# parsaeskandar/pangenome-index

Hardware: AMD Instinct MI355X
Metric: find_mems reads/sec (150 bp batch) (higher is better)
Workload: dtype u64

## Files before the change

pangenome-index_amd/csrc/pgx_image.h:

```cpp
#ifndef PGX_IMAGE_H
#define PGX_IMAGE_H

#include <stdint.h>

#define PGX_IMAGE_LAYOUT 1u

#define PGX_BLOCK_BYTES 64
#define PGX_BLOCK_RUNS 16
#define PGX_RUN_LEN_BITS 12
#define PGX_RUN_LEN_MAX 4095u
#define PGX_COUNT_BITS 40
#define PGX_DIR_MAX_SHIFT 12
#define PGX_IMAGE_RL 0u
#define PGX_IMAGE_DENSE 1u
#define PGX_IMAGE_DENSE2 2u
#define PGX_D2_SYMS 384u
#define PGX_D2_BLOCK_BYTES 128u
#define PGX_PAIRS_SYMS 96u
#define PGX_PAIRS_BLOCK_BYTES 128u
#define PGX_PAIRS_STRIDE64 64u
#define PGX_SB_MAX 64u
#define PGX_D2_SB_SHIFT 22u
#define PGX_PAIRS_SB_SHIFT 24u

#define PGX_EXT_CV(e) ((e) & 7u)
#define PGX_EXT_V(e) (((e) >> 3) & 7u)
#define PGX_EXT_M(e) (((e) >> 6) & 0x3FFFFu)
#define PGX_EXT_KILL(e) (((e) >> 24) & 1u)
#define PGX_EXT_MAKE(cv, v, m, kill) \
    ((uint32_t)(cv) | ((uint32_t)(v) << 3) | ((uint32_t)(m) << 6) | ((uint32_t)(kill) << 24))

typedef struct {
    uint64_t n;
    uint64_t C[8];
    uint32_t ext_tab[512];
    uint32_t slot_code[8];
    uint32_t sigma;
    uint32_t excl_mask;
    uint32_t dir_shift;
    uint32_t n_blocks;
    uint64_t dir_entries;
    uint64_t n_tag_runs;
    uint64_t tag_dir_entries;
    uint32_t tag_dir_shift;
    uint32_t has_tags;
    uint32_t mode;
    uint32_t count_supported;
    uint32_t cnt_tab[256];
    uint32_t image_kind;
    uint32_t has_pairs;
    uint32_t pair_t2[32];
    uint32_t pair_runs;
    uint32_t reserved1;
    uint32_t wide;
    uint32_t d2_sb_shift, pairs_sb_shift;
    uint32_t n_sb2, n_sbp;
    uint32_t pairs_stride;
    uint64_t pair_t2w[32];
} PgxConsts;

#define PGX_NO_POSITION (~(uint64_t)0)
typedef struct {
    uint64_t n;
    uint64_t n_runs;
    uint64_t n_last;
    uint64_t max_length;
    uint64_t rdir_entries, ldir_entries;
    uint32_t rdir_shift, ldir_shift;
} PgxLocConsts;

// ... 2 lines not shown
```

pangenome-index_amd/csrc/pgx_index.cpp:

```cpp
#include <algorithm>
#include <cstdio>
#include <cstdlib>
#include <array>
#include <cstring>
#include <memory>
#include <mutex>
#include <thread>

#include "pgx_host.hpp"

namespace pgx {

static thread_local std::string g_last_error;
void set_last_error(const std::string &m) { g_last_error = m; }
const std::string &last_error() { return g_last_error; }

static inline unsigned bytecode_len(uint64_t v) {
    unsigned k = 1;
    while (v > 0x7F) { v >>= 7; k++; }
    return k;
}

void RiFile::parse(const uint8_t *p, uint64_t n) {
    ByteReader r(p, n);
// ... 306 lines not shown
static void build_dense_image(const RiFile &ri, HostImage &img) {
    PgxConsts &c = img.consts;
    const uint64_t nb = (c.n >> 6) + 1;
    if (nb >> 32) throw Error(PGX_ERR_UNSUPPORTED, "BWT too long for the dense image");
    img.blocks.assign(nb * PGX_BLOCK_BYTES, 0);
    img.bstart.clear();
    img.dir.assign(1, 0);
    img.blow.clear();
    uint32_t *dw = reinterpret_cast<uint32_t *>(img.blocks.data());
    uint64_t c6[6] = {0, 0, 0, 0, 0, 0};
    auto put_header = [&](uint64_t b) {
        uint32_t *h = dw + b * 16;
        for (int i = 0; i < 6; i++) h[i] = (uint32_t)c6[i];
        for (int i = 0; i < 4; i++) h[6] |= (uint32_t)((c6[i] >> 32) & 0xFF) << (8 * i);
        h[7] = (uint32_t)((c6[4] >> 32) & 0xFF) | ((uint32_t)((c6[5] >> 32) & 0xFF) << 8);
    };
    uint64_t pos = 0, n_runs = 0;
    put_header(0);
    for (const auto &blk : ri.blocks)
        for (const auto &ru : blk.runs) {
            n_runs++;
            const uint32_t code = ru.first;
            uint64_t left = ru.second;
            while (left) {
                const uint64_t b = pos >> 6;
                const uint32_t off = (uint32_t)(pos & 63);
                const uint64_t take = std::min<uint64_t>(left, 64 - off);
                const uint64_t bits = (take == 64 ? ~0ull : ((1ull << take) - 1ull)) << off;
                uint32_t *h = dw + b * 16;
                for (int p = 0; p < 3; p++)
                    if ((code >> p) & 1u) {
                        h[8 + 2 * p] |= (uint32_t)bits;
                        h[9 + 2 * p] |= (uint32_t)(bits >> 32);
                    }
                c6[code] += take;
                left -= take;
                pos += take;
                if ((pos & 63) == 0) put_header(pos >> 6);
            }
        }
    if (pos != c.n) throw Error(PGX_ERR_FORMAT, "FastLocate: run lengths do not add up to the BWT size");
    img.n_runs = n_runs;
    c.n_blocks = (uint32_t)nb;
    c.dir_shift = 0;
    c.dir_entries = 1;
    c.image_kind = PGX_IMAGE_DENSE;
}

static uint32_t sb_shift_for(uint64_t nb, uint32_t want) {
    uint32_t sh = want;
    while (((nb - 1) >> sh) + 1 > PGX_SB_MAX) sh++;
    return sh;
}
static void build_dense2_image(const RiFile &ri, HostImage &img, bool wide, uint32_t sb_shift_want) {
    PgxConsts &c = img.consts;
    if ((c.n >> 32) && !wide) throw Error(PGX_ERR_UNSUPPORTED, "BWT too long for the narrow dense2 image");
    const uint64_t nb = c.n / PGX_D2_SYMS + 1;
    if (nb >> 32) throw Error(PGX_ERR_UNSUPPORTED, "BWT too long for the dense2 image");
    const uint32_t sb_shift = wide ? sb_shift_for(nb, sb_shift_want) : 31u;
    if (wide && (PGX_D2_SYMS << sb_shift) > (1ull << 31)) throw Error(PGX_ERR_UNSUPPORTED, "BWT too long for the wide dense2 image (more than PGX_SB_MAX superblocks)");
    const uint64_t n_sb = wide ? ((nb - 1) >> sb_shift) + 1 : 1;
    img.sbase2.assign(n_sb * 8, 0);
    uint64_t base[6] = {0, 0, 0, 0, 0, 0};
    img.blocks.assign(nb * PGX_D2_BLOCK_BYTES, 0);
    img.bstart.clear();
    img.dir.assign(1, 0);
    img.blow.clear();
    img.exc.clear();
    uint32_t *dw = reinterpret_cast<uint32_t *>(img.blocks.data());
    uint64_t c6[6] = {0, 0, 0, 0, 0, 0};
    static const int hdr_slot[6] = {-1, 0, 1, 2, 4, 3};
    static const int two_bit[6] = {0, 0, 1, 2, 0, 3};
    auto put_header = [&](uint64_t b) {
        uint32_t *h = dw + b * 32;
        if (wide && (b & ((1ull << sb_shift) - 1)) == 0) {
            uint64_t *sb = img.sbase2.data() + (b >> sb_shift) * 8;
            uint64_t sum = 0;
            for (int i = 1; i < 6; i++) { base[i] = c6[i]; sb[hdr_slot[i]] = c6[i]; sum += c6[i]; }
            sb[5] = sum;
        }
        for (int i = 1; i < 6; i++) h[hdr_slot[i]] = (uint32_t)(c6[i] - base[i]);
        if (img.exc.size() >> 24) throw Error(PGX_ERR_UNSUPPORTED, "too many exception runs for the dense2 image");
        h[5] = (uint32_t)img.exc.size();
    };
    auto set_bits = [](uint32_t *words, uint32_t lo, uint32_t hi) {
        for (uint32_t w = lo >> 5; w <= ((hi - 1) >> 5); w++) {
            const uint32_t a = std::max(lo, w << 5) & 31u, e = std::min(hi, (w + 1) << 5) - (w << 5);
            words[w] |= (e == 32 ? 0xFFFFFFFFu : ((1u << e) - 1u)) & ~((1u << a) - 1u);
        }
    };
    auto finish_block = [&](uint64_t b) {
        uint32_t *h = dw + b * 32;
        uint64_t sub = 0;
        uint32_t n0 = 0, n1 = 0, n3 = 0;
        for (int s = 0; s < 2; s++) {
            for (int k = 0; k < 4; k++) {
                const uint32_t a = h[8 + 8 * s + k], d = h[12 + 8 * s + k];
                n0 += (uint32_t)__builtin_popcount(a); n1 += (uint32_t)__builtin_popcount(d); n3 += (uint32_t)__builtin_popcount(a & d);
            }
            sub |= ((uint64_t)n0 | ((uint64_t)n1 << 9) | ((uint64_t)n3 << 18)) << (27 * s);
        }
        h[6] = (uint32_t)sub; h[7] = (uint32_t)(sub >> 32);
    };
    uint64_t pos = 0, n_runs = 0;
    put_header(0);
    for (const auto &blk : ri.blocks)
        for (const auto &ru : blk.runs) {
            n_runs++;
            const uint32_t code = ru.first;
            uint64_t left = ru.second;
            while (left) {
                const uint64_t b = pos / PGX_D2_SYMS;
                const uint32_t off = (uint32_t)(pos % PGX_D2_SYMS);
                const uint64_t take = std::min<uint64_t>(left, PGX_D2_SYMS - off);
                uint32_t *h = dw + b * 32;
                const int tb = two_bit[code];
                if (tb)
                    for (uint32_t i = off; i < off + (uint32_t)take;) {
                        uint32_t *sb = h + 8 + 8 * (i >> 7);
                        const uint32_t lo = i & 127u, hi = std::min<uint32_t>(128u, lo + (off + (uint32_t)take - i));
                        if (tb & 1) set_bits(sb, lo, hi);
                        if (tb & 2) set_bits(sb + 4, lo, hi);
                        i += hi - lo;
                    }
                if (code == 0 || code == 4) {
                    const uint32_t kind = code == 4 ? 1u : 0u;
                    if ((h[5] >> 24) && (img.exc.back() >> 18) == kind && (img.exc.back() & 511u) + ((img.exc.back() >> 9) & 511u) == off)
                        img.exc.back() += (uint32_t)take << 9;
                    else {
                        img.exc.push_back(off | ((uint32_t)take << 9) | (kind << 18));
                        h[5] += 1u << 24;
                    }
                }
                c6[code] += take;
                left -= take;
                pos += take;
                if (pos % PGX_D2_SYMS == 0) { finish_block(b); put_header(pos / PGX_D2_SYMS); }
            }
        }
    if (pos != c.n) throw Error(PGX_ERR_FORMAT, "FastLocate: run lengths do not add up to the BWT size");
    finish_block(nb - 1);
    if (img.exc.empty()) img.exc.push_back(0);
    img.n_runs = n_runs;
    c.n_blocks = (uint32_t)nb;
    c.dir_shift = 0;
    c.dir_entries = 1;
    c.image_kind = PGX_IMAGE_DENSE2;
    c.wide = wide ? 1u : 0u;
    c.d2_sb_shift = sb_shift;
    c.n_sb2 = (uint32_t)n_sb;
}

static bool build_pairs_image(const RiFile &ri, HostImage &img, bool wide, uint32_t sb_shift_want, uint32_t stride) {
    if (stride != PGX_PAIRS_SYMS && stride != PGX_PAIRS_STRIDE64) return false;
    PgxConsts &c = img.consts;
// ... 196 lines not shown
        if (const char *e = std::getenv("PGX_IMAGE")) {
            const std::string v(e);
            force = v == "dense" ? PGX_MODE_IMAGE_DENSE : v == "dense2" ? PGX_MODE_IMAGE_DENSE2 : v == "rl" ? PGX_MODE_IMAGE_RL : v == "pairs" ? PGX_MODE_IMAGE_PAIRS : 0u;
            if (v == "wide" || v == "wide-pairs") { wide = true; force = PGX_MODE_IMAGE_PAIRS; }
            if (v == "wide-dense2") { wide = true; force = PGX_MODE_IMAGE_DENSE2; }
        }
    if (force & (force - 1)) throw Error(PGX_ERR_ARG, "pgx_index_open: more than one image layout forced");
    if (wide && (force & (PGX_MODE_IMAGE_RL | PGX_MODE_IMAGE_DENSE))) throw Error(PGX_ERR_ARG, "pgx_index_open: PGX_MODE_IMAGE_WIDE goes with dense2 / pairs only");
    if (wide && !force) force = PGX_MODE_IMAGE_PAIRS;
    const bool fits_wide = c.n < ((uint64_t)PGX_SB_MAX << 30);
    if (force & (PGX_MODE_IMAGE_DENSE | PGX_MODE_IMAGE_DENSE2 | PGX_MODE_IMAGE_PAIRS)) {
        if (!can) throw Error(PGX_ERR_UNSUPPORTED, "dense image: not available for a legacy-layout index without N in COMPAT mode");
        if ((force & (PGX_MODE_IMAGE_DENSE2 | PGX_MODE_IMAGE_PAIRS)) && (c.n >> 32)) {
            if (!fits_wide) throw Error(PGX_ERR_UNSUPPORTED, "dense2 image: BWT too long");
            wide = true;
        }
        if (force & PGX_MODE_IMAGE_PAIRS) pairs = wide && !(mode_bits & PGX_MODE_IMAGE_PAIRS) && !std::getenv("PGX_IMAGE") ? 1 : 2;
        return (force & PGX_MODE_IMAGE_DENSE) ? PGX_IMAGE_DENSE : PGX_IMAGE_DENSE2;
    }
    if ((force & PGX_MODE_IMAGE_RL) || !can) return PGX_IMAGE_RL;
    const uint64_t dense_blocks = (c.n >> 6) + 1;
    if (dense_blocks * 80 + 16 <= 48 * 1024) return PGX_IMAGE_DENSE;
    const uint64_t dense_bytes0 = dense_blocks * PGX_BLOCK_BYTES;
    if (dense_bytes0 <= (224ull << 20)) { pairs = (c.n >> 32) ? 0 : 1; return PGX_IMAGE_DENSE; }
    if (!(c.n >> 32)) { pairs = 1; return PGX_IMAGE_DENSE2; }
    if (fits_wide) { pairs = 1; wide = true; return PGX_IMAGE_DENSE2; }
    uint64_t runs = 0;
    for (const auto &b : ri.blocks) runs += b.runs.size();
    const uint64_t dense_bytes = dense_blocks * PGX_BLOCK_BYTES, rl_bytes = (runs / PGX_BLOCK_RUNS + 1) * (PGX_BLOCK_BYTES + 4);
    const uint64_t cache = 192ull << 20;
    return (rl_bytes > cache && dense_bytes <= (64ull << 30)) ? PGX_IMAGE_DENSE : PGX_IMAGE_RL;
}

void build_rank_image(const RiFile &ri, uint32_t mode_bits, HostImage &img) {
    const uint32_t mode = mode_bits & PGX_MODE_MASK;
    PgxConsts &c = img.consts;
    std::memset(&c, 0, sizeof c);
    c.n = ri.sequence_size;
    c.mode = mode;
    build_ext_tables(ri, mode, c);
    build_count_table(ri, mode, c);
    int pairs = 0;
    bool wide = false;
    const uint32_t kind = choose_image(ri, mode_bits, c, pairs, wide);
    img.pairs.clear(); img.sbase2.clear(); img.pbase.clear();
    uint32_t sh2 = PGX_D2_SB_SHIFT, shp = PGX_PAIRS_SB_SHIFT;
    if (const char *e = std::getenv("PGX_SB_SHIFT")) { sh2 = (uint32_t)std::min<unsigned long>(std::strtoul(e, nullptr, 10), PGX_D2_SB_SHIFT); shp = sh2 + 2; }
    uint32_t pstride = (2 * c.n <= (64ull << 30)) ? PGX_PAIRS_STRIDE64 : PGX_PAIRS_SYMS;
    if (const char *e = std::getenv("PGX_PAIRS_STRIDE")) {
        const unsigned long v = std::strtoul(e, nullptr, 10);
        if (v == PGX_PAIRS_SYMS) pstride = PGX_PAIRS_SYMS;
        else if (v == PGX_PAIRS_STRIDE64) pstride = PGX_PAIRS_STRIDE64;
    }
    if (kind == PGX_IMAGE_DENSE) {
        build_dense_image(ri, img);
        if (pairs) (void)build_pairs_image(ri, img, false, shp, pstride);
        return;
    }
    if (kind == PGX_IMAGE_DENSE2) {
        build_dense2_image(ri, img, wide, sh2);
        if (pairs && !build_pairs_image(ri, img, wide, shp, pstride) && pairs == 2)
            throw Error(PGX_ERR_UNSUPPORTED, "pairs image: the index does not qualify (extension tables of a COMPAT quirk, or too many N / endmarker runs)");
        return;
    }
    const bool refine = c.excl_mask != 0;
    img.blocks.clear();
    img.bstart.clear();
    uint64_t c6[6] = {0, 0, 0, 0, 0, 0};
    uint64_t head[6];
    std::vector<std::pair<uint8_t, uint32_t>> ent;
    uint64_t pos = 0, block_pos = 0, E = 0, n_runs = 0;
    auto open_block = [&]() {
        for (int i = 0; i < 6; i++) head[i] = (c.excl_mask >> i) & 1 ? E : c6[i];
        block_pos = pos;
        ent.clear();
    };
    auto close_block = [&]() {
        if (ent.empty()) return;
        put_block(img.blocks, head, ent);
        img.bstart.push_back(block_pos);
        ent.clear();
    };
    open_block();
    for (uint64_t b = 0; b < ri.blocks.size(); b++) {
        if (refine) {
            close_block();
            E = ri.blocks[b].cum[0];
            open_block();
        }
        for (auto &ru : ri.blocks[b].runs) {
            n_runs++;
            uint64_t left = ru.second;
            while (left) {
                if (!ent.empty() && ent.back().first == ru.first && ent.back().second < PGX_RUN_LEN_MAX) {
                    uint32_t add = (uint32_t)std::min<uint64_t>(left, PGX_RUN_LEN_MAX - ent.back().second);
                    ent.back().second += add;
                    left -= add; pos += add; c6[ru.first] += add;
                    continue;
                }
                if (ent.size() == PGX_BLOCK_RUNS) { close_block(); open_block(); }
                uint32_t take = (uint32_t)std::min<uint64_t>(left, PGX_RUN_LEN_MAX);
                ent.emplace_back(ru.first, take);
                left -= take; pos += take; c6[ru.first] += take;
            }
        }
    }
    close_block();
    if (img.bstart.empty()) {
        uint64_t z[6] = {0};
        put_block(img.blocks, z, {});
        img.bstart.push_back(0);
    }
    img.n_runs = n_runs;
// ... 394 lines not shown
```

pangenome-index_amd/csrc/pgx_pairs_kernels.hip:

```cpp
#include <hip/hip_runtime.h>
#include <stdint.h>

#include <type_traits>

#include "pgx_device.h"
#include "pgx_rank_device.h"
#include "pgx_slots_device.h"

#ifndef PGX_PAIRS_PACKED_WAVES
#define PGX_PAIRS_PACKED_WAVES 5
#endif
#ifndef PGX_LCE_WAVES
#define PGX_LCE_WAVES PGX_FM_WAVES_PER_SIMD
#endif
#ifndef PGX_LCE_ENTRY_CAP
#define PGX_LCE_ENTRY_CAP 3u
#endif
#define PGX_PK_GROUP 12u

__device__ __forceinline__ uint32_t pgx_window_byte(uint64_t w0, uint64_t w1, uint64_t a) {
    return (uint32_t)(((a & 8ull) ? w1 : w0) >> (8u * (uint32_t)(a & 7ull))) & 0xFFu;
}
__device__ __forceinline__ uint32_t pgx_packed_seed_index(const uint32_t *s_rd, uint32_t rd_stride, uint32_t q, int32_t K) {
    const uint32_t w0 = s_rd[(q >> 4) * rd_stride + threadIdx.x], w1 = s_rd[((q >> 4) + 1u) * rd_stride + threadIdx.x];
// ... 432 lines not shown
                const int32_t ta = (int32_t)relA - 32 * h, tb = (int32_t)relB - 32 * h;
                const uint32_t mP = ta >= 32 ? 0xFFFFFFFFu : (ta > 0 ? ((1u << ta) - 1u) : 0u);
                const uint32_t mR = (tb >= 32 ? 0xFFFFFFFFu : (tb > 0 ? ((1u << tb) - 1u) : 0u)) & ~mP;
                const uint32_t x = PX[h], y = PY[h], u = PU[h], v = PV[h];
                const uint32_t m1 = (x ^ i0) & (y ^ i1);
                const uint32_t g1 = (y & ua) | (x & (y | va) & wa);
                const uint32_t q2 = m1 & (u ^ j0) & (v ^ j1);
                const uint32_t g2 = m1 & ((v & ub) | (u & (v | vb) & wb));
                e1p += __popc(m1 & mP); e2p += __popc(q2 & mP);
                e1r += __popc(m1 & mR); g1r += __popc(g1 & mR); e2r += __popc(q2 & mR); g2r += __popc(g2 & mR);
            }
            pos_t a01 = (pos_t)(row.x + row.y + row.z + row.w + pts + e1p);
            pos_t a02 = (pos_t)((t2 == 0u ? row.x : (t2 == 1u ? row.y : (t2 == 2u ? row.z : row.w))) + e2p);
            if (WIDE) {
                const uint64_t *pb = s_pb + (size_t)((bfirst + pend) >> pa.pairs_sb_shift) * 24u;
                a01 += (pos_t)pb[16u + t1];
                a02 += (pos_t)pb[4u * t1 + t2];
            }
            const bool straddle = endrel > SYMS, far = endrel > STRIDE + SYMS;
            const uint32_t over = endrel - SYMS;
            const bool cont2 = !pend && straddle && over <= (hs.y >> 24), cont1 = !pend && straddle && !cont2 && over <= (hs.z >> 24);
            const bool cont = cont1 || cont2;
            if (cont) {
                const uint32_t l1 = (PX[2] >> 31) | ((PY[2] >> 31) << 1), l2 = (PU[2] >> 31) | ((PV[2] >> 31) << 1);
                e1r += l1 == t1 ? over : 0u;
                g1r += l1 > t1 ? over : 0u;
                e2r += (cont2 && l1 == t1 && l2 == t2) ? over : 0u;
                g2r += (cont2 && l1 == t1 && l2 > t2) ? over : 0u;
            }
            const bool bail = !fr && (flagged || (far && !cont));
            const bool wait = !fr && !pend && straddle && !bail && !cont;
#ifdef PGX_FM_STATS
            st_wait += wait ? 1ull : 0ull;
#endif
            if (wait) {
                X0 = e1r | (g1r << 8) | (e2r << 16) | (g2r << 24); X0e = a01; X0f = a02;
                pend = 1u;
            } else {
                const uint32_t Xp = pend ? X0 : 0u;
                const uint32_t c1 = (Xp & 0xFFu) + e1r, w1 = ((Xp >> 8) & 0xFFu) + g1r, c2 = ((Xp >> 16) & 0xFFu) + e2r, w2 = (Xp >> 24) + g2r;
                const pos_t r1 = pend ? X0e : a01, r2 = pend ? X0f : a02;
                pend = 0u;
                pos_t s1 = reg1 ? (pos_t)c1 : (pos_t)0;
                pos_t k1 = r1 + s_C[PGX_EXT_V(e1)], q1v = kq + (pos_t)w1;
                if (bail) {
                    const uint64_t q0 = (uint64_t)p0 > (uint64_t)n ? (uint64_t)n : (uint64_t)p0, q1 = (uint64_t)p1 > (uint64_t)n ? (uint64_t)n : (uint64_t)p1;
                    uint64_t A0 = 0, A1 = 0, B0 = 0, B1 = 0;
                    PgxDevImage img = {};
                    img.blocks = PGX_PAIRS_COLD(blocks); img.exc = PGX_PAIRS_COLD(exc); img.sbase2 = PGX_PAIRS_COLD(sbase2); img.d2_sb_shift = PGX_PAIRS_COLD(d2_sb_shift);
#pragma unroll 1
                    for (int it = 0; it < 2; it++) {
                        const uint64_t q = it ? q1 : q0;
                        uint64_t a, bq;
                        if (WIDE) pgx_dense2w_rank(img, q, PGX_EXT_CV(e1), PGX_EXT_M(e1), a, bq);
                        else if (pa.dense == 1) {
                            const PgxDenseBlk db = pgx_dense_load<false>(img, nullptr, q);
                            pgx_dense_rank(db, q, PGX_EXT_CV(e1), PGX_EXT_M(e1), a, bq);
                        } else pgx_dense2_rank(img, (uint32_t)q, PGX_EXT_CV(e1), PGX_EXT_M(e1), a, bq);
                        A1 = a; B1 = bq;
                        if (!it) { A0 = a; B0 = bq; }
                    }
                    const uint64_t dB = B1 - B0;
                    {
                        const unsigned long long here = __ballot(true);
                        if (lane == (int)__ffsll((long long)here) - 1) {
                            atomicAdd(PGX_PAIRS_COLD(ctr) + PGX_CTR_REDO, (unsigned long long)__popcll(here));
                            atomicAdd(PGX_PAIRS_COLD(ctr) + PGX_CTR_PAIRS_LINES, 2ull * (unsigned long long)__popcll(here));
                        }
                    }
                    const bool none = PGX_EXT_KILL(e1) || A0 >= A1;
                    s1 = none ? (pos_t)0 : (pos_t)(A1 - A0);
                    k1 = (pos_t)A0 + s_C[PGX_EXT_V(e1)];
                    q1v = kq + (pos_t)dB;
                }
                if (fr) { const uint4 f = s_fe[PACKED ? (at_end ? 4u : ((byte >> 1) & 3u)) : byte]; k1 = ent_k(f); q1v = ent_q(f); s1 = ent_s(f); }
                const bool small1 = s1 == 0u || s1 < mo || mo_huge;
                const uint32_t sdepth = se.w >> 24;
                const pos_t se_s = ent_s(se);
                const bool seed_alive = seed_lane && se_s != 0u && se_s >= mo && !mo_huge;
                const bool seed_dead = seed_lane && se_s == 0u && sdepth != PGX_SEED_UNUSABLE && mo <= 1u;
                const bool do2 = (fr ? (at_end && rem2 && have2 && !seed_alive && !seed_dead) : (two && !bail && !cont1)) && !small1;
                pos_t s2 = (pos_t)c2, k2 = r2 + s_C[PGX_EXT_V(e2)] + s_t2[8u * t1 + cv2], q2v = q1v + (pos_t)w2;
                if (fr) { const uint4 f = s_fe[PACKED ? 5u + ((byte2 >> 1) & 3u) : 256u + byte2]; k2 = ent_k(f); q2v = ent_q(f); s2 = ent_s(f); }
                pos_t ns = do2 ? s2 : s1, nk = do2 ? k2 : k1, nq = do2 ? q2v : q1v;
                if (ns == 0u) { nk = 0u; nq = 0u; }
                if (do2) {
                    Jk = fwd ? q1v : Jk;
                    Js = fwd ? s1 : Js;
                    j = fwd ? j + 1 : j - 1;
                }
                next += do2 ? 2u : 1u;
                did2 = do2 ? 1u : 0u;
                s = ns;
                k = fwd ? nq : nk;
                kp = fwd ? nk : nq;
                bool small = ns == 0u || ns < mo || mo_huge;
                if (seed_alive) {
                    k = ent_k(se); kp = ent_q(se); s = se_s;
                    small = false;
                    j -= (int32_t)kuse - 1;
                    next += kuse - 1u;
                } else if (seed_dead) {
                    k = 0u; kp = 0u; s = 0u;
                    small = true;
                    j -= (int32_t)sdepth - 1;
                    next += sdepth - 1u;
                }
                const bool adv = !small, q1 = ph == 1, q2 = ph == 2, at_x = j == x;
                const bool to2 = q1 && adv && at_x;
                const bool keep = adv && (to2 || q2);
                Jk = keep ? k : Jk;
// ... 120 lines not shown
```

pangenome-index_amd/csrc/pgx_rank_device.h:

```cpp
#pragma once

#include <hip/hip_runtime.h>
#include <stdint.h>

#include "pgx_device.h"

template <bool LDS_IMAGE>
__device__ __forceinline__ uint32_t pgx_find_block(const PgxDevImage &img, const uint64_t *__restrict__ lds_dir,
                                                   const uint16_t *__restrict__ lds_blow, uint64_t pos) {
    const uint64_t di = pos >> img.dir_shift;
    const uint64_t e = LDS_IMAGE ? lds_dir[di] : img.dir[di];
    const uint32_t lowp = (uint32_t)pos & ((1u << img.dir_shift) - 1u);
    uint32_t lo = (uint32_t)e;
    const uint32_t cnt = (uint32_t)(e >> 32) & 0xFFu;
    if (cnt <= 2) {
        const uint32_t l0 = (uint32_t)(e >> 40) & 0xFFFu, l1 = (uint32_t)(e >> 52);
        return lo - 1u + ((cnt >= 1 && l0 <= lowp) ? 1u : 0u) + ((cnt >= 2 && l1 <= lowp) ? 1u : 0u);
    }
    uint32_t hi = cnt < 255 ? lo + cnt : (uint32_t)(LDS_IMAGE ? lds_dir[di + 1] : img.dir[di + 1]);
    while (lo < hi) {
        const uint32_t mid = (lo + hi) >> 1;
        const uint32_t v = LDS_IMAGE ? lds_blow[mid] : img.blow[mid];
        if (v <= lowp) lo = mid + 1; else hi = mid;
    }
// ... 44 lines not shown
        ia = (cv == (uint32_t)i) ? t[i] : ia;
        const uint32_t w = (mrow >> (3 * i)) & 7u;
        b += c[i] * (uint64_t)w;
        ib += t[i] * w;
    }
    A = a + ia;
    B = b + ib;
}

__device__ __forceinline__ void pgx_dense_inblock(const PgxDenseBlk &blk, uint32_t pos_lo, uint32_t t[6]) {
    const uint32_t rel = pos_lo & 63u;
    const uint32_t mlo = rel >= 32u ? 0xFFFFFFFFu : ((1u << rel) - 1u);
    const uint32_t mhi = rel > 32u ? ((1u << (rel - 32u)) - 1u) : 0u;
    const uint32_t a0 = blk.p01.x & mlo, a1 = blk.p01.y & mhi, b0 = blk.p01.z & mlo, b1 = blk.p01.w & mhi;
    const uint32_t d0 = blk.p2.x & mlo, d1 = blk.p2.y & mhi;
    const uint32_t n1 = __popc(a0) + __popc(a1), n2 = __popc(b0) + __popc(b1), n4 = __popc(d0) + __popc(d1);
    const uint32_t n3 = __popc(a0 & b0) + __popc(a1 & b1), n5 = __popc(a0 & d0) + __popc(a1 & d1);
    t[3] = n3; t[5] = n5;
    t[1] = n1 - n3 - n5; t[2] = n2 - n3; t[4] = n4 - n5;
    t[0] = rel - (n1 + n2 + n4 - n3 - n5);
}

__device__ __forceinline__ void pgx_dense_pair32(const PgxDenseBlk &k0, uint32_t p0, const PgxDenseBlk &k1, uint32_t p1, uint32_t cv,
                                                 uint32_t mrow, uint32_t &A0, uint32_t &A1, uint32_t &dB) {
    uint32_t t0[6], t1[6];
    pgx_dense_inblock(k0, p0, t0);
    pgx_dense_inblock(k1, p1, t1);
    const uint32_t c0[6] = {k0.h0.x + t0[0], k0.h0.y + t0[1], k0.h0.z + t0[2], k0.h0.w + t0[3], k0.h1.x + t0[4], k0.h1.y + t0[5]};
    const uint32_t c1[6] = {k1.h0.x + t1[0], k1.h0.y + t1[1], k1.h0.z + t1[2], k1.h0.w + t1[3], k1.h1.x + t1[4], k1.h1.y + t1[5]};
    uint32_t a0 = 0, a1 = 0, d = 0;
#pragma unroll
    for (int i = 0; i < 6; i++) {
        a0 = (cv == (uint32_t)i) ? c0[i] : a0;
        a1 = (cv == (uint32_t)i) ? c1[i] : a1;
        d += (c1[i] - c0[i]) * ((mrow >> (3 * i)) & 7u);
    }
    A0 = a0; A1 = a1; dB = d;
}

struct PgxDense2Blk {
    uint4 h0, h1;
    uint4 p0, p1;
};
__device__ __forceinline__ PgxDense2Blk pgx_dense2_load(const PgxDevImage &img, uint32_t pos, uint32_t &rel) {
    const uint32_t blk = (uint32_t)(((uint64_t)pos * 0xAAAAAAABull) >> 40);
    rel = pos - blk * PGX_D2_SYMS;
    const uint4 *bp = img.blocks + (size_t)blk * 8;
    PgxDense2Blk b;
    b.h0 = bp[0]; b.h1 = bp[1];
    const uint4 *sp = bp + 2 + 2 * (rel >> 7);
    b.p0 = sp[0]; b.p1 = sp[1];
    return b;
}
__device__ __forceinline__ void pgx_dense2_counts(const PgxDevImage &img, const PgxDense2Blk &b, uint32_t pos, uint32_t rel, uint32_t c[6]) {
    const uint32_t sub = rel >> 7, r = rel & 127u;
    const uint64_t sc = ((uint64_t)b.h1.z | ((uint64_t)b.h1.w << 32)) >> (sub == 2u ? 27 : 0);
    uint32_t n0 = sub ? (uint32_t)sc & 511u : 0u, n1 = sub ? (uint32_t)(sc >> 9) & 511u : 0u, n3 = sub ? (uint32_t)(sc >> 18) & 511u : 0u;
    const uint32_t a[4] = {b.p0.x, b.p0.y, b.p0.z, b.p0.w}, d[4] = {b.p1.x, b.p1.y, b.p1.z, b.p1.w};
#pragma unroll
    for (int h = 0; h < 4; h++) {
        const int32_t t = (int32_t)r - 32 * h;
        const uint32_t m = t >= 32 ? 0xFFFFFFFFu : (t > 0 ? ((1u << t) - 1u) : 0u);
        const uint32_t x = a[h] & m, y = d[h] & m;
        n0 += __popc(x); n1 += __popc(y); n3 += __popc(x & y);
    }
    uint32_t e0 = 0, e4 = 0;
    const uint32_t ec = b.h1.y >> 24;
    if (ec) {
        const uint32_t *ep = img.exc + (b.h1.y & 0xFFFFFFu);
        for (uint32_t i = 0; i < ec; i++) {
            const uint32_t u = ep[i], st = u & 511u, ln = (u >> 9) & 511u;
            const uint32_t cnt = rel > st ? min(rel - st, ln) : 0u;
            if ((u >> 18) & 1u) e4 += cnt; else e0 += cnt;
        }
    }
    const uint32_t hsum = b.h0.x + b.h0.y + b.h0.z + b.h0.w + b.h1.x;
    c[0] = (pos - rel) - hsum + e0;
    c[1] = b.h0.x + rel - (n0 + n1 - n3) - e0 - e4;
    c[2] = b.h0.y + n0 - n3;
    c[3] = b.h0.z + n1 - n3;
    c[4] = b.h1.x + e4;
    c[5] = b.h0.w + n3;
}
template <bool NARROW>
__device__ __forceinline__ void pgx_dense2_pair(const PgxDevImage &img, uint32_t p0, uint32_t p1, uint32_t cv, uint32_t mrow, uint64_t &A0, uint64_t &A1,
                                                uint64_t &dB, bool lower = true) {
    uint32_t r0, r1;
    const PgxDense2Blk k0 = pgx_dense2_load(img, p0, r0), k1 = pgx_dense2_load(img, p1, r1);
    if (lower) __builtin_amdgcn_s_setprio(0);
    uint32_t c0[6], c1[6];
    pgx_dense2_counts(img, k0, p0, r0, c0);
    pgx_dense2_counts(img, k1, p1, r1, c1);
    uint32_t a0 = 0, a1 = 0, d32 = 0;
    uint64_t d64 = 0;
#pragma unroll
    for (int i = 0; i < 6; i++) {
        a0 = (cv == (uint32_t)i) ? c0[i] : a0;
        a1 = (cv == (uint32_t)i) ? c1[i] : a1;
        const uint32_t w = (mrow >> (3 * i)) & 7u;
        if (NARROW) d32 += (c1[i] - c0[i]) * w;
        else d64 += (uint64_t)((int64_t)c1[i] - (int64_t)c0[i]) * (uint64_t)w;
    }
    A0 = a0; A1 = a1; dB = NARROW ? (uint64_t)d32 : d64;
}
__device__ __forceinline__ void pgx_dense2_rank(const PgxDevImage &img, uint32_t pos, uint32_t cv, uint32_t mrow, uint64_t &A, uint64_t &B) {
    uint32_t rel;
    const PgxDense2Blk k = pgx_dense2_load(img, pos, rel);
    uint32_t c[6];
    pgx_dense2_counts(img, k, pos, rel, c);
    uint64_t a = 0, bb = 0;
#pragma unroll
    for (int i = 0; i < 6; i++) {
        a = (cv == (uint32_t)i) ? (uint64_t)c[i] : a;
        bb += (uint64_t)c[i] * (uint64_t)((mrow >> (3 * i)) & 7u);
    }
    A = a; B = bb;
}

template <bool MULHI = false>
__device__ __forceinline__ PgxDense2Blk pgx_dense2w_load(const PgxDevImage &img, uint64_t pos, uint32_t &rel, uint32_t &blk) {
    blk = MULHI ? (uint32_t)(__umul64hi(pos, 0xAAAAAAAAAAAAAAABull) >> 8)
                : (uint32_t)(((pos >> 7) * 0xAAAAAAABull) >> 33);
    rel = (uint32_t)(pos - (uint64_t)blk * PGX_D2_SYMS);
    const uint4 *bp = img.blocks + (size_t)blk * 8;
    PgxDense2Blk b;
    b.h0 = bp[0]; b.h1 = bp[1];
    const uint4 *sp = bp + 2 + 2 * (rel >> 7);
    b.p0 = sp[0]; b.p1 = sp[1];
    return b;
}
__device__ __forceinline__ void pgx_dense2w_counts(const PgxDevImage &img, const uint64_t *__restrict__ sb, const PgxDense2Blk &b, uint64_t pos, uint32_t rel,
                                                   uint32_t blk, uint64_t c[6]) {
    uint32_t d[6];
    pgx_dense2_counts(img, b, rel, rel, d);
    const uint64_t *base = sb + (size_t)(blk >> img.d2_sb_shift) * 8;
    c[0] = (pos - rel) - base[5] + (uint64_t)(int64_t)(int32_t)d[0];
    c[1] = base[0] + d[1];
    c[2] = base[1] + d[2];
    c[3] = base[2] + d[3];
    c[4] = base[4] + d[4];
    c[5] = base[3] + d[5];
}
__device__ __forceinline__ void pgx_dense2w_pair(const PgxDevImage &img, const uint64_t *__restrict__ sb, uint64_t p0, uint64_t p1, uint32_t cv, uint32_t mrow,
                                                 uint64_t &A0, uint64_t &A1, uint64_t &dB, bool lower = true) {
    uint32_t r0, r1, b0, b1;
    const PgxDense2Blk k0 = pgx_dense2w_load(img, p0, r0, b0), k1 = pgx_dense2w_load(img, p1, r1, b1);
    if (lower) __builtin_amdgcn_s_setprio(0);
    uint64_t c0[6], c1[6];
    pgx_dense2w_counts(img, sb, k0, p0, r0, b0, c0);
    pgx_dense2w_counts(img, sb, k1, p1, r1, b1, c1);
    uint64_t a0 = 0, a1 = 0, d = 0;
#pragma unroll
    for (int i = 0; i < 6; i++) {
        a0 = (cv == (uint32_t)i) ? c0[i] : a0;
        a1 = (cv == (uint32_t)i) ? c1[i] : a1;
        d += (c1[i] - c0[i]) * (uint64_t)((mrow >> (3 * i)) & 7u);
    }
    A0 = a0; A1 = a1; dB = d;
}
template <bool MULHI = false>
__device__ __forceinline__ void pgx_dense2w_rank(const PgxDevImage &img, uint64_t pos, uint32_t cv, uint32_t mrow, uint64_t &A, uint64_t &B) {
    uint32_t rel, blk;
    const PgxDense2Blk k = pgx_dense2w_load<MULHI>(img, pos, rel, blk);
    uint64_t c[6];
    pgx_dense2w_counts(img, img.sbase2, k, pos, rel, blk, c);
    uint64_t a = 0, bb = 0;
#pragma unroll
    for (int i = 0; i < 6; i++) {
        a = (cv == (uint32_t)i) ? c[i] : a;
        bb += c[i] * (uint64_t)((mrow >> (3 * i)) & 7u);
    }
    A = a; B = bb;
}

template <bool LDS_IMAGE>
__device__ __forceinline__ void pgx_rank_ab(const PgxDevImage &img, const uint4 *__restrict__ lds_blocks,
                                            const uint64_t *__restrict__ lds_dir, const uint16_t *__restrict__ lds_blow,
                                            uint64_t pos, uint32_t cv, uint32_t mrow, uint64_t &A, uint64_t &B) {
    if (pos > img.n) pos = img.n;
    if (img.dense == 3) { pgx_dense2w_rank(img, pos, cv, mrow, A, B); return; }
    if (img.dense == 2) { pgx_dense2_rank(img, (uint32_t)pos, cv, mrow, A, B); return; }
    if (img.dense) {
        pgx_dense_rank(pgx_dense_load<LDS_IMAGE>(img, lds_blocks, pos), pos, cv, mrow, A, B);
        return;
    }
    const uint32_t lo = pgx_find_block<LDS_IMAGE>(img, lds_dir, lds_blow, pos);
    const uint4 *bp = (LDS_IMAGE ? lds_blocks : img.blocks) + (size_t)lo * 4;
    const uint4 h0 = bp[0], h1 = bp[1], r0 = bp[2], r1 = bp[3];
    uint64_t c[6];
    c[0] = (uint64_t)h0.x | ((uint64_t)(h1.z & 0xFFu) << 32);
    c[1] = (uint64_t)h0.y | ((uint64_t)((h1.z >> 8) & 0xFFu) << 32);
    c[2] = (uint64_t)h0.z | ((uint64_t)((h1.z >> 16) & 0xFFu) << 32);
    c[3] = (uint64_t)h0.w | ((uint64_t)(h1.z >> 24) << 32);
    c[4] = (uint64_t)h1.x | ((uint64_t)(h1.w & 0xFFu) << 32);
    c[5] = (uint64_t)h1.y | ((uint64_t)((h1.w >> 8) & 0xFFu) << 32);
    uint64_t start = 0, a = 0, b = 0;
#pragma unroll
    for (int i = 0; i < 6; i++) {
        start += ((img.excl_mask >> i) & 1u) ? 0ull : c[i];
        a = (cv == (uint32_t)i) ? c[i] : a;
        b += c[i] * (uint64_t)((mrow >> (3 * i)) & 7u);
    }
    uint32_t rel = (uint32_t)(pos - start);
    uint32_t ia = 0, ib = 0;
    const uint32_t arow = 1u << (3 * cv);
    const uint32_t rw[8] = {r0.x, r0.y, r0.z, r0.w, r1.x, r1.y, r1.z, r1.w};
#pragma unroll
    for (int e = 0; e < PGX_BLOCK_RUNS; e++) {
        const uint32_t w = rw[e >> 1];
        const uint32_t sh = (e & 1) ? (w >> 28) : __builtin_amdgcn_ubfe(w, 12, 4);
        const uint32_t len = (e & 1) ? __builtin_amdgcn_ubfe(w, 16, 12) : (w & PGX_RUN_LEN_MAX);
        const uint32_t take = min(len, rel);
        rel -= take;
        ia += take * __builtin_amdgcn_ubfe(arow, sh, 3);
        ib += take * __builtin_amdgcn_ubfe(mrow, sh, 3);
    }
    A = a + ia;
    B = b + ib;
// ... 147 lines not shown
```

Baseline: 1.163 billion.

## Add dense2 exception hint bit and batch exception-list fetches in rank

```diff
diff --git a/pangenome-index_amd/csrc/pgx_image.h b/pangenome-index_amd/csrc/pgx_image.h
--- a/pangenome-index_amd/csrc/pgx_image.h
+++ b/pangenome-index_amd/csrc/pgx_image.h
@@ -16,6 +16,10 @@
 #define PGX_IMAGE_DENSE2 2u
 #define PGX_D2_SYMS 384u
 #define PGX_D2_BLOCK_BYTES 128u
+#define PGX_D2_HINT_BIT 0x80000000u
+#define PGX_D2_HINT_Q(w) (((w) >> 22) & 511u)
+#define PGX_D2_HINT_NONE 511u
+#define PGX_D2_EXC_BATCH 8u
 #define PGX_PAIRS_SYMS 96u
 #define PGX_PAIRS_BLOCK_BYTES 128u
 #define PGX_PAIRS_STRIDE64 64u
diff --git a/pangenome-index_amd/csrc/pgx_index.cpp b/pangenome-index_amd/csrc/pgx_index.cpp
--- a/pangenome-index_amd/csrc/pgx_index.cpp
+++ b/pangenome-index_amd/csrc/pgx_index.cpp
@@ -382,7 +382,7 @@
     while (((nb - 1) >> sh) + 1 > PGX_SB_MAX) sh++;
     return sh;
 }
-static void build_dense2_image(const RiFile &ri, HostImage &img, bool wide, uint32_t sb_shift_want) {
+static void build_dense2_image(const RiFile &ri, HostImage &img, bool wide, uint32_t sb_shift_want, bool exc_hint) {
     PgxConsts &c = img.consts;
     if ((c.n >> 32) && !wide) throw Error(PGX_ERR_UNSUPPORTED, "BWT too long for the narrow dense2 image");
     const uint64_t nb = c.n / PGX_D2_SYMS + 1;
@@ -431,6 +431,21 @@
             sub |= ((uint64_t)n0 | ((uint64_t)n1 << 9) | ((uint64_t)n3 << 18)) << (27 * s);
         }
         h[6] = (uint32_t)sub; h[7] = (uint32_t)(sub >> 32);
+        const uint32_t ec = h[5] >> 24;
+        if (!exc_hint || !ec || b + 1 >= nb) return;
+        const uint32_t *ep = img.exc.data() + (h[5] & 0xFFFFFFu);
+        uint32_t n_len = 0, q = PGX_D2_HINT_NONE, end = 0;
+        for (uint32_t i = 0; i < ec; i++) {
+            const uint32_t st = ep[i] & 511u, ln = (ep[i] >> 9) & 511u;
+            if (!((ep[i] >> 18) & 1u)) return;
+            if (st > end) q = end;
+            n_len += ln;
+            end = st + ln;
+        }
+        if (end < PGX_D2_SYMS) q = end;
+        if (n_len == PGX_D2_SYMS) q = PGX_D2_HINT_NONE;
+        else if (n_len != PGX_D2_SYMS - 1u) return;
+        h[7] |= PGX_D2_HINT_BIT | (q << 22);
     };
     uint64_t pos = 0, n_runs = 0;
     put_header(0);
@@ -733,13 +748,14 @@
         if (v == PGX_PAIRS_SYMS) pstride = PGX_PAIRS_SYMS;
         else if (v == PGX_PAIRS_STRIDE64) pstride = PGX_PAIRS_STRIDE64;
     }
+    const bool exc_hint = !(std::getenv("PGX_D2_EXC_HINT") && std::getenv("PGX_D2_EXC_HINT")[0] == '0');
     if (kind == PGX_IMAGE_DENSE) {
         build_dense_image(ri, img);
         if (pairs) (void)build_pairs_image(ri, img, false, shp, pstride);
         return;
     }
     if (kind == PGX_IMAGE_DENSE2) {
-        build_dense2_image(ri, img, wide, sh2);
+        build_dense2_image(ri, img, wide, sh2, exc_hint);
         if (pairs && !build_pairs_image(ri, img, wide, shp, pstride) && pairs == 2)
             throw Error(PGX_ERR_UNSUPPORTED, "pairs image: the index does not qualify (extension tables of a COMPAT quirk, or too many N / endmarker runs)");
         return;
diff --git a/pangenome-index_amd/csrc/pgx_pairs_kernels.hip b/pangenome-index_amd/csrc/pgx_pairs_kernels.hip
--- a/pangenome-index_amd/csrc/pgx_pairs_kernels.hip
+++ b/pangenome-index_amd/csrc/pgx_pairs_kernels.hip
@@ -508,11 +508,11 @@
                     for (int it = 0; it < 2; it++) {
                         const uint64_t q = it ? q1 : q0;
                         uint64_t a, bq;
-                        if (WIDE) pgx_dense2w_rank(img, q, PGX_EXT_CV(e1), PGX_EXT_M(e1), a, bq);
+                        if (WIDE) pgx_dense2w_rank<false, false>(img, q,PGX_EXT_CV(e1), PGX_EXT_M(e1), a, bq);
                         else if (pa.dense == 1) {
                             const PgxDenseBlk db = pgx_dense_load<false>(img, nullptr, q);
                             pgx_dense_rank(db, q, PGX_EXT_CV(e1), PGX_EXT_M(e1), a, bq);
-                        } else pgx_dense2_rank(img, (uint32_t)q, PGX_EXT_CV(e1), PGX_EXT_M(e1), a, bq);
+                        } else pgx_dense2_rank<false>(img, (uint32_t)q, PGX_EXT_CV(e1), PGX_EXT_M(e1), a, bq);
                         A1 = a; B1 = bq;
                         if (!it) { A0 = a; B0 = bq; }
                     }
diff --git a/pangenome-index_amd/csrc/pgx_rank_device.h b/pangenome-index_amd/csrc/pgx_rank_device.h
--- a/pangenome-index_amd/csrc/pgx_rank_device.h
+++ b/pangenome-index_amd/csrc/pgx_rank_device.h
@@ -120,10 +120,39 @@
     b.p0 = sp[0]; b.p1 = sp[1];
     return b;
 }
-__device__ __forceinline__ void pgx_dense2_counts(const PgxDevImage &img, const PgxDense2Blk &b, uint32_t pos, uint32_t rel, uint32_t c[6]) {
+struct PgxD2Exc {
+    uint32_t u[PGX_D2_EXC_BATCH];
+};
+__device__ __forceinline__ bool pgx_dense2_needs_exc(const PgxDense2Blk &b) { return (b.h1.y >> 24) != 0u && !(b.h1.w & PGX_D2_HINT_BIT); }
+__device__ __forceinline__ void pgx_dense2_exc_fetch(const PgxDevImage &img, const PgxDense2Blk &b, PgxD2Exc &x) {
+    const uint32_t last = (b.h1.y >> 24) - 1u;
+    const uint32_t *ep = img.exc + (b.h1.y & 0xFFFFFFu);
+#pragma unroll
+    for (uint32_t i = 0; i < PGX_D2_EXC_BATCH; i++) x.u[i] = ep[min(i, last)];
+}
+__device__ __forceinline__ void pgx_dense2_exc_add(uint32_t u, uint32_t rel, uint32_t &e0, uint32_t &e4) {
+    const uint32_t st = u & 511u, ln = (u >> 9) & 511u;
+    const uint32_t cnt = rel > st ? min(rel - st, ln) : 0u;
+    if ((u >> 18) & 1u) e4 += cnt; else e0 += cnt;
+}
+__device__ __forceinline__ void pgx_dense2_exc_counts(const PgxDevImage &img, const PgxDense2Blk &b, uint32_t rel, const PgxD2Exc &x, uint32_t &e0, uint32_t &e4) {
+    e0 = 0; e4 = 0;
+    const uint32_t ec = b.h1.y >> 24;
+    if (!ec) return;
+    if (b.h1.w & PGX_D2_HINT_BIT) {
+        e4 = rel - (rel > PGX_D2_HINT_Q(b.h1.w) ? 1u : 0u);
+        return;
+    }
+    const uint32_t *ep = img.exc + (b.h1.y & 0xFFFFFFu);
+#pragma unroll
+    for (uint32_t i = 0; i < PGX_D2_EXC_BATCH; i++)
+        if (i < ec) pgx_dense2_exc_add(x.u[i], rel, e0, e4);
+    for (uint32_t i = PGX_D2_EXC_BATCH; i < ec; i++) pgx_dense2_exc_add(ep[i], rel, e0, e4);
+}
+__device__ __forceinline__ void pgx_dense2_inblock(const PgxDense2Blk &b, uint32_t rel, uint32_t &n0, uint32_t &n1, uint32_t &n3) {
     const uint32_t sub = rel >> 7, r = rel & 127u;
     const uint64_t sc = ((uint64_t)b.h1.z | ((uint64_t)b.h1.w << 32)) >> (sub == 2u ? 27 : 0);
-    uint32_t n0 = sub ? (uint32_t)sc & 511u : 0u, n1 = sub ? (uint32_t)(sc >> 9) & 511u : 0u, n3 = sub ? (uint32_t)(sc >> 18) & 511u : 0u;
+    n0 = sub ? (uint32_t)sc & 511u : 0u; n1 = sub ? (uint32_t)(sc >> 9) & 511u : 0u; n3 = sub ? (uint32_t)(sc >> 18) & 511u : 0u;
     const uint32_t a[4] = {b.p0.x, b.p0.y, b.p0.z, b.p0.w}, d[4] = {b.p1.x, b.p1.y, b.p1.z, b.p1.w};
 #pragma unroll
     for (int h = 0; h < 4; h++) {
@@ -132,16 +161,9 @@
         const uint32_t x = a[h] & m, y = d[h] & m;
         n0 += __popc(x); n1 += __popc(y); n3 += __popc(x & y);
     }
-    uint32_t e0 = 0, e4 = 0;
-    const uint32_t ec = b.h1.y >> 24;
-    if (ec) {
-        const uint32_t *ep = img.exc + (b.h1.y & 0xFFFFFFu);
-        for (uint32_t i = 0; i < ec; i++) {
-            const uint32_t u = ep[i], st = u & 511u, ln = (u >> 9) & 511u;
-            const uint32_t cnt = rel > st ? min(rel - st, ln) : 0u;
-            if ((u >> 18) & 1u) e4 += cnt; else e0 += cnt;
-        }
-    }
+}
+__device__ __forceinline__ void pgx_dense2_sums(const PgxDense2Blk &b, uint32_t pos, uint32_t rel, uint32_t n0, uint32_t n1, uint32_t n3, uint32_t e0, uint32_t e4,
+                                                uint32_t c[6]) {
     const uint32_t hsum = b.h0.x + b.h0.y + b.h0.z + b.h0.w + b.h1.x;
     c[0] = (pos - rel) - hsum + e0;
     c[1] = b.h0.x + rel - (n0 + n1 - n3) - e0 - e4;
@@ -150,15 +172,55 @@
     c[4] = b.h1.x + e4;
     c[5] = b.h0.w + n3;
 }
+__device__ __forceinline__ void pgx_dense2_counts_e(const PgxDense2Blk &b, uint32_t pos, uint32_t rel, uint32_t e0, uint32_t e4, uint32_t c[6]) {
+    uint32_t n0, n1, n3;
+    pgx_dense2_inblock(b, rel, n0, n1, n3);
+    pgx_dense2_sums(b, pos, rel, n0, n1, n3, e0, e4, c);
+}
+template <bool BATCH = true>
+__device__ __forceinline__ void pgx_dense2_counts(const PgxDevImage &img, const PgxDense2Blk &b, uint32_t pos, uint32_t rel, uint32_t c[6]) {
+    uint32_t e0 = 0, e4 = 0;
+    if (BATCH) {
+        PgxD2Exc x = {};
+        if (pgx_dense2_needs_exc(b)) pgx_dense2_exc_fetch(img, b, x);
+        pgx_dense2_exc_counts(img, b, rel, x, e0, e4);
+        pgx_dense2_counts_e(b, pos, rel, e0, e4, c);
+        return;
+    }
+    uint32_t n0, n1, n3;
+    pgx_dense2_inblock(b, rel, n0, n1, n3);
+    const bool hint = (b.h1.w & PGX_D2_HINT_BIT) != 0u;
+    const uint32_t ec = hint ? 0u : b.h1.y >> 24;
+    e4 = hint ? rel - (rel > PGX_D2_HINT_Q(b.h1.w) ? 1u : 0u) : 0u;
+    if (ec) {
+        const uint32_t *ep = img.exc + (b.h1.y & 0xFFFFFFu);
+        for (uint32_t i = 0; i < ec; i++) pgx_dense2_exc_add(ep[i], rel, e0, e4);
+    }
+    pgx_dense2_sums(b, pos, rel, n0, n1, n3, e0, e4, c);
+}
+__device__ __forceinline__ void pgx_dense2_pair_exc(const PgxDevImage &img, const PgxDense2Blk &k0, uint32_t r0, const PgxDense2Blk &k1, uint32_t r1, bool same,
+                                                    uint32_t &e00, uint32_t &e04, uint32_t &e10, uint32_t &e14) {
+    e00 = 0; e04 = 0; e10 = 0; e14 = 0;
+    if ((k0.h1.y | k1.h1.y) >> 24) {
+        PgxD2Exc x0 = {}, x1 = {};
+        const bool n0 = pgx_dense2_needs_exc(k0), n1 = pgx_dense2_needs_exc(k1);
+        if (n0) pgx_dense2_exc_fetch(img, k0, x0);
+        if (n1 && !same) pgx_dense2_exc_fetch(img, k1, x1);
+        if (same) x1 = x0;
+        pgx_dense2_exc_counts(img, k0, r0, x0, e00, e04);
+        pgx_dense2_exc_counts(img, k1, r1, x1, e10, e14);
+    }
+}
 template <bool NARROW>
 __device__ __forceinline__ void pgx_dense2_pair(const PgxDevImage &img, uint32_t p0, uint32_t p1, uint32_t cv, uint32_t mrow, uint64_t &A0, uint64_t &A1,
                                                 uint64_t &dB, bool lower = true) {
     uint32_t r0, r1;
     const PgxDense2Blk k0 = pgx_dense2_load(img, p0, r0), k1 = pgx_dense2_load(img, p1, r1);
     if (lower) __builtin_amdgcn_s_setprio(0);
-    uint32_t c0[6], c1[6];
-    pgx_dense2_counts(img, k0, p0, r0, c0);
-    pgx_dense2_counts(img, k1, p1, r1, c1);
+    uint32_t c0[6], c1[6], e00, e04, e10, e14;
+    pgx_dense2_pair_exc(img, k0, r0, k1, r1, p0 - r0 == p1 - r1, e00, e04, e10, e14);
+    pgx_dense2_counts_e(k0, p0, r0, e00, e04, c0);
+    pgx_dense2_counts_e(k1, p1, r1, e10, e14, c1);
     uint32_t a0 = 0, a1 = 0, d32 = 0;
     uint64_t d64 = 0;
 #pragma unroll
@@ -171,11 +233,12 @@
     }
     A0 = a0; A1 = a1; dB = NARROW ? (uint64_t)d32 : d64;
 }
+template <bool BATCH = true>
 __device__ __forceinline__ void pgx_dense2_rank(const PgxDevImage &img, uint32_t pos, uint32_t cv, uint32_t mrow, uint64_t &A, uint64_t &B) {
     uint32_t rel;
     const PgxDense2Blk k = pgx_dense2_load(img, pos, rel);
     uint32_t c[6];
-    pgx_dense2_counts(img, k, pos, rel, c);
+    pgx_dense2_counts<BATCH>(img, k, pos, rel, c);
     uint64_t a = 0, bb = 0;
 #pragma unroll
     for (int i = 0; i < 6; i++) {
@@ -197,10 +260,8 @@
     b.p0 = sp[0]; b.p1 = sp[1];
     return b;
 }
-__device__ __forceinline__ void pgx_dense2w_counts(const PgxDevImage &img, const uint64_t *__restrict__ sb, const PgxDense2Blk &b, uint64_t pos, uint32_t rel,
-                                                   uint32_t blk, uint64_t c[6]) {
-    uint32_t d[6];
-    pgx_dense2_counts(img, b, rel, rel, d);
+__device__ __forceinline__ void pgx_dense2w_widen(const PgxDevImage &img, const uint64_t *__restrict__ sb, const uint32_t d[6], uint64_t pos, uint32_t rel, uint32_t blk,
+                                                  uint64_t c[6]) {
     const uint64_t *base = sb + (size_t)(blk >> img.d2_sb_shift) * 8;
     c[0] = (pos - rel) - base[5] + (uint64_t)(int64_t)(int32_t)d[0];
     c[1] = base[0] + d[1];
@@ -209,14 +270,26 @@
     c[4] = base[4] + d[4];
     c[5] = base[3] + d[5];
 }
+template <bool BATCH = true>
+__device__ __forceinline__ void pgx_dense2w_counts(const PgxDevImage &img, const uint64_t *__restrict__ sb, const PgxDense2Blk &b, uint64_t pos, uint32_t rel,
+                                                   uint32_t blk, uint64_t c[6]) {
+    uint32_t d[6];
+    pgx_dense2_counts<BATCH>(img, b, rel, rel, d);
+    pgx_dense2w_widen(img, sb, d, pos, rel, blk, c);
+}
 __device__ __forceinline__ void pgx_dense2w_pair(const PgxDevImage &img, const uint64_t *__restrict__ sb, uint64_t p0, uint64_t p1, uint32_t cv, uint32_t mrow,
                                                  uint64_t &A0, uint64_t &A1, uint64_t &dB, bool lower = true) {
     uint32_t r0, r1, b0, b1;
     const PgxDense2Blk k0 = pgx_dense2w_load(img, p0, r0, b0), k1 = pgx_dense2w_load(img, p1, r1, b1);
     if (lower) __builtin_amdgcn_s_setprio(0);
     uint64_t c0[6], c1[6];
-    pgx_dense2w_counts(img, sb, k0, p0, r0, b0, c0);
-    pgx_dense2w_counts(img, sb, k1, p1, r1, b1, c1);
+    uint32_t e00, e04, e10, e14;
+    pgx_dense2_pair_exc(img, k0, r0, k1, r1, b0 == b1, e00, e04, e10, e14);
+    uint32_t d0[6], d1[6];
+    pgx_dense2_counts_e(k0, r0, r0, e00, e04, d0);
+    pgx_dense2_counts_e(k1, r1, r1, e10, e14, d1);
+    pgx_dense2w_widen(img, sb, d0, p0, r0, b0, c0);
+    pgx_dense2w_widen(img, sb, d1, p1, r1, b1, c1);
     uint64_t a0 = 0, a1 = 0, d = 0;
 #pragma unroll
     for (int i = 0; i < 6; i++) {
@@ -226,12 +299,12 @@
     }
     A0 = a0; A1 = a1; dB = d;
 }
-template <bool MULHI = false>
+template <bool MULHI = false, bool BATCH = true>
 __device__ __forceinline__ void pgx_dense2w_rank(const PgxDevImage &img, uint64_t pos, uint32_t cv, uint32_t mrow, uint64_t &A, uint64_t &B) {
     uint32_t rel, blk;
     const PgxDense2Blk k = pgx_dense2w_load<MULHI>(img, pos, rel, blk);
     uint64_t c[6];
-    pgx_dense2w_counts(img, img.sbase2, k, pos, rel, blk, c);
+    pgx_dense2w_counts<BATCH>(img, img.sbase2, k, pos, rel, blk, c);
     uint64_t a = 0, bb = 0;
 #pragma unroll
     for (int i = 0; i < 6; i++) {
```

New measurement: 1.166 billion, median of 6. Within noise of the previous version (+0.3%).
